# 6Lackiu/EMplanner_Carla

Hardware: AMD Instinct MI355X
Metric: planning cycles/sec (DP+QP, 40x9 S-L lattice, 8 obs) (higher is better)
Workload: dtype f64

## Files before the change

emplanner_carla_amd/csrc/emp_frenet_core.h:

```cpp
#pragma once

#include "emp_core.h"

#if !defined(__HIPCC__)
#include <algorithm>
#endif

namespace emp {

#if !defined(__HIPCC__)
using std::max;
using std::min;
#endif

struct Node {
    double x, y, theta, kappa;
};
EMP_HD Node node_at(const double* line, int i) { return Node{line[4 * i], line[4 * i + 1], line[4 * i + 2], line[4 * i + 3]}; }

EMP_HD int match_scan(const double* line, int n_ref, double x, double y, int first, int step, int limit) {
    int match = 0, worse = 0;
    double best = __builtin_inf();
    for (int i = first; i >= 0 && i < n_ref; i += step) {
        const double dx = line[4 * i] - x, dy = line[4 * i + 1] - y;
        const double d = sqrt(dx * dx + dy * dy);
        if (d < best) {
            best = d;
            match = i;
            worse = 0;
        } else if (++worse >= limit) {
            break;
        }
    }
    return match;
}

EMP_HD double dot2(double a0, double a1, double b0, double b1) { return __builtin_fma(a1, b1, a0 * b0); }

EMP_HD void sincos_pair(double x, double* s, double* c) {
#if defined(__HIP_DEVICE_COMPILE__)
    sincos(x, s, c);
#else
    *s = sin(x);
    *c = cos(x);
#endif
}

EMP_HD Node node_advanced(const Node& m, double ds, double c, double s) {
    return Node{m.x + ds * c, m.y + ds * s, m.theta + m.kappa * ds, m.kappa};
}
EMP_HD void normal_offset(double x, double y, double l, double c, double s, double* ox, double* oy) {
    *ox = x + l * (-s);
    *oy = y + l * c;
}

EMP_HD Node project_on_cs(const Node& m, double c, double s, double x, double y) {
    return node_advanced(m, dot2(x - m.x, y - m.y, c, s), c, s);
}
EMP_HD Node project_on(const Node& m, double x, double y) {
    double c, s;
    sincos_pair(m.theta, &s, &c);
    return project_on_cs(m, c, s, x, y);
}
EMP_HD double projection_s_cs(const Node& m, double c, double s, double s_at_m, double x, double y) {
    return s_at_m + dot2(x - m.x, y - m.y, c, s);
}

EMP_HD double projection_s(const Node& m, double s_at_m, double x, double y) {
    double c, sn;
    sincos_pair(m.theta, &sn, &c);
    return s_at_m + dot2(x - m.x, y - m.y, c, sn);
}

EMP_HD double lateral_offset(const Node& proj, double x, double y) {
    double c, s;
    sincos_pair(proj.theta, &s, &c);
    return dot2(x - proj.x, y - proj.y, -s, c);
}
EMP_HD double lateral_offset_cs(const Node& proj, double c, double s, double x, double y) {
    return dot2(x - proj.x, y - proj.y, -s, c);
}

EMP_HD void s_map_build(const double* line, int n_ref, double ox, double oy, double* s_map) {
    const int m0 = match_scan(line, n_ref, ox, oy, 0, 1, 50);
    double acc = 0.0;
    s_map[0] = 0.0;
    for (int i = 1; i < n_ref; ++i) {
        const double dx = line[4 * i] - line[4 * (i - 1)], dy = line[4 * i + 1] - line[4 * (i - 1) + 1];
        acc = sqrt(dx * dx + dy * dy) + acc;
        s_map[i] = acc;
    }
    const double s0 = projection_s(node_at(line, m0), s_map[m0], ox, oy);
    for (int i = 0; i < n_ref; ++i) s_map[i] = s_map[i] - s0;
}

struct FrenetState {
    double l, l_dot, s_dot, l_ddot, dl_ds, s_ddot, ddl_ds;
};
EMP_HD FrenetState frenet_state_cs(const Node& proj, double c, double s, double px, double py, double vx, double vy, double ax,
                                   double ay) {
    FrenetState o;
    const double k = proj.kappa;
    o.l = dot2(px - proj.x, py - proj.y, -s, c);
    o.l_dot = dot2(vx, vy, -s, c);
    o.s_dot = dot2(vx, vy, c, s) / (1.0 - k * o.l);
    o.l_ddot = dot2(ax, ay, -s, c) - k * (1.0 - k * o.l) * (o.s_dot * o.s_dot);
    o.dl_ds = (fabs(o.s_dot) < 1e-6) ? 0.0 : o.l_dot / o.s_dot;
    o.s_ddot = (dot2(ax, ay, c, s) + 2.0 * (o.s_dot * o.s_dot * k * o.dl_ds) + o.s_dot * o.s_dot * 0.0 * o.l) / (1.0 - k * o.l);
    o.ddl_ds = (fabs(o.s_dot) < 1e-6) ? 0.0 : (o.l_ddot - o.dl_ds * o.s_ddot) / (o.s_dot * o.s_dot);
    return o;
}
EMP_HD FrenetState frenet_state(const Node& proj, double px, double py, double vx, double vy, double ax, double ay) {
    double c, s;
    sincos_pair(proj.theta, &s, &c);
    return frenet_state_cs(proj, c, s, px, py, vx, vy, ax, ay);
}

EMP_HD bool proj_point(const double* line, const double* s_map, int n_ref, double s, int* idx, Node* out) {
    int i = *idx;
    while (true) {
        if (i + 1 >= n_ref) return false;
        if (!(s_map[i + 1] < s)) break;
        ++i;
    }
    const Node m = node_at(line, i);
    const double ds = s - s_map[i];
    double c, sn;
    sincos_pair(m.theta, &sn, &c);
    *out = node_advanced(m, ds, c, sn);
    *idx = i;
    return true;
}

EMP_HD int walk_from_zero(const double* sm, int P, double s, bool* off_end) {
    int lo = 0, hi = P - 1;
    while (lo < hi) {
        const int mid = (lo + hi) >> 1;
        if (sm[mid + 1] < s) lo = mid + 1;
        else hi = mid;
    }
    *off_end = lo + 1 >= P;
    return lo;
}

EMP_HD int argmin_abs(const double* s, int stride, int n, double target) {
    int best = 0;
    double bv = fabs(s[0] - target);
    for (int j = 1; j < n; ++j) {
        const double v = fabs(s[j * stride] - target);
        if (v < bv) {
            bv = v;
            best = j;
        }
    }
    return best;
}

EMP_HD void argmin_abs3(const double* s, int n, double t0, double t1, double t2, int* i0, int* i1, int* i2) {
    const double f = s[0];
    double b0 = fabs(f - t0), b1 = fabs(f - t1), b2 = fabs(f - t2);
    int k0 = 0, k1 = 0, k2 = 0;
    for (int j0 = 1; j0 < n; j0 += 4) {
        double v[4];
#pragma unroll
        for (int u = 0; u < 4; ++u) v[u] = s[min(j0 + u, n - 1)];
#pragma unroll
        for (int u = 0; u < 4; ++u) {
            const int j = j0 + u;
            const double a0 = fabs(v[u] - t0), a1 = fabs(v[u] - t1), a2 = fabs(v[u] - t2);
            if (a0 < b0) { b0 = a0; k0 = j; }
            if (a1 < b1) { b1 = a1; k1 = j; }
            if (a2 < b2) { b2 = a2; k2 = j; }
        }
    }
    *i0 = min(k0, n - 1);
    *i1 = min(k1, n - 1);
    *i2 = min(k2, n - 1);
}

EMP_HD bool lmin_lmax(const double* dp_s, const double* dp_l, int stride, int n, const double* obs_s,
                                 const double* obs_l, int n_obs, double obs_length, double obs_width, double* l_min,
                                 double* l_max) {
    for (int j = 0; j < n; ++j) {
        l_min[j] = -10.0;
        l_max[j] = 10.0;
    }
    for (int k = 0; k < n_obs; ++k) {
        const int lo = argmin_abs(dp_s, stride, n, obs_s[k] - obs_length / 2.0) + 2;
        const int hi = argmin_abs(dp_s, stride, n, obs_s[k] + obs_length / 2.0) + 2;
        const int centre = argmin_abs(dp_s, stride, n, obs_s[k]);
        const bool below = dp_l[centre * stride] < obs_l[k];
        for (int j = lo; j <= hi; ++j) {
            if (j >= n) return false;
            if (below) l_max[j] = fmin(l_max[j], obs_l[k] - obs_width / 2.0);
            else l_min[j] = fmax(l_min[j], obs_l[k] + obs_width / 2.0);
        }
    }
    return true;
}

EMP_HD double centred_diff(const double* v, int stride, int i, int m) {
    const int a = (i - 1 > 0) ? i - 1 : 0, b = (i < m - 2) ? i : m - 2;
    return ((v[(a + 1) * stride] - v[a * stride]) + (v[(b + 1) * stride] - v[b * stride])) / 2.0;
}

EMP_HD void heading_kappa(const double* xy, int stride, int m, double* theta, int tstride, double* kappa, int kstride) {
    for (int i = 0; i < m; ++i) {
        const double dx = centred_diff(xy, stride, i, m), dy = centred_diff(xy + 1, stride, i, m);
        theta[i * tstride] = atan2(dy, dx);
    }
    for (int i = 0; i < m; ++i) {
        const double dx = centred_diff(xy, stride, i, m), dy = centred_diff(xy + 1, stride, i, m);
        kappa[i * kstride] = sin(centred_diff(theta, tstride, i, m)) / sqrt(dx * dx + dy * dy);
    }
}

}
```

emplanner_carla_amd/csrc/emp_qp_rows.h:

```cpp
#pragma once

#include "emp_qp_wave.h"

#ifndef EMP_QP_DEBUG_ROWS
#define EMP_QP_DEBUG_ROWS(...)
#endif

namespace emp {

#pragma clang fp contract(fast)

template <int GP, class Op>
__device__ __forceinline__ double oct_reduce(double v, Op op) {
    static_assert(GP == 8 || GP == 16, "groups of 8 or 16 lanes");
    v = op(v, dpp_move<0xB1>(v));
    v = op(v, dpp_move<0x4E>(v));
    v = op(v, dpp_move<0x141>(v));
    if constexpr (GP == 16) v = op(v, dpp_move<0x140>(v));
    return v;
}
template <int GP>
__device__ __forceinline__ double oct_max(double v) { return oct_reduce<GP>(v, [](double a, double b) { return vmax(a, b); }); }
template <int GP>
__device__ __forceinline__ double oct_min(double v) { return oct_reduce<GP>(v, [](double a, double b) { return vmin(a, b); }); }
// ... 116 lines not shown
        for (int e = 1; e <= KD; ++e) p[e] = lane_up1(y[R - e]);
#pragma unroll
        for (int r = 0; r < R; ++r) {
            double acc = rhs[r];
#pragma unroll
            for (int e = 1; e <= KD; ++e) acc = __builtin_fma(-low[r][e], (r >= e) ? y[r - e] : p[e - r], acc);
            y[r] = acc * rinv[r];
        }
    }
    double x[R];
#pragma unroll
    for (int r = 0; r < R; ++r) x[r] = y[r] * rinv[r];
    for (int k = 0; k < steps; ++k) {
        double q[KD + 1];
#pragma unroll
        for (int e = 1; e <= KD; ++e) q[e] = lane_dn1(x[e - 1]);
#pragma unroll
        for (int r = R - 1; r >= 0; --r) {
            double acc = y[r];
#pragma unroll
            for (int e = 1; e <= KD; ++e) acc = __builtin_fma(-a[r][e], (r + e < R) ? x[r + e] : q[r + e - R + 1], acc);
            x[r] = acc * rinv[r];
        }
    }
#pragma unroll
    for (int r = 0; r < R; ++r) b[r] = x[r];
}

template <int GP, int R>
__device__ __forceinline__ bool band_chol_rows3(double (&a)[R][4], double (&rinv)[R], double (&low)[R][4], int N, int gl,
                                               bool active, int steps) {
    static_assert(R >= 3, "a lane must hold at least KD = 3 rows");
    double A[R][4];
    bool rowv[R], inband[R][4];
#pragma unroll
    for (int r = 0; r < R; ++r) {
        const int j = gl * R + r;
        rowv[r] = active && j < N;
#pragma unroll
        for (int d = 0; d < 4; ++d) {
            A[r][d] = rowv[r] ? a[r][d] : (d == 0 ? 1.0 : 0.0);
            a[r][d] = A[r][d];
            inband[r][d] = rowv[r] && j + d < N;
        }
        rinv[r] = 1.0;
    }
    double diag[R];
    for (int k = 0; k < steps; ++k) {
        const double n1_1 = lane_up1(a[R - 1][1]), n1_2 = lane_up1(a[R - 1][2]), n1_3 = lane_up1(a[R - 1][3]);
        const double n2_2 = lane_up1(a[R - 2][2]), n2_3 = lane_up1(a[R - 2][3]);
        const double n3_3 = lane_up1(a[R - 3][3]);
#pragma unroll
        for (int r = 0; r < R; ++r) {
            double u1_1, u1_2, u1_3, u2_2, u2_3, u3_3;
            if (r >= 1) { u1_1 = a[r - 1][1]; u1_2 = a[r - 1][2]; u1_3 = a[r - 1][3]; }
            else        { u1_1 = n1_1; u1_2 = n1_2; u1_3 = n1_3; }
            if (r >= 2)      { u2_2 = a[r - 2][2]; u2_3 = a[r - 2][3]; }
            else if (r == 1) { u2_2 = n1_2; u2_3 = n1_3; }
            else             { u2_2 = n2_2; u2_3 = n2_3; }
            if (r >= 3)      u3_3 = a[r - 3][3];
            else if (r == 2) u3_3 = n1_3;
            else if (r == 1) u3_3 = n2_3;
            else             u3_3 = n3_3;
            double acc0 = A[r][0], acc1 = A[r][1], acc2 = A[r][2];
            const double acc3 = A[r][3];
            acc0 = __builtin_fma(-u1_1, u1_1, acc0);
            acc1 = __builtin_fma(-u1_1, u1_2, acc1);
            acc2 = __builtin_fma(-u1_1, u1_3, acc2);
            acc0 = __builtin_fma(-u2_2, u2_2, acc0);
            acc1 = __builtin_fma(-u2_2, u2_3, acc1);
            acc0 = __builtin_fma(-u3_3, u3_3, acc0);
            diag[r] = acc0;
            const double rs = fast_rsqrt(acc0 > 0.0 ? acc0 : 1.0);
            a[r][0] = acc0 * rs;
            a[r][1] = inband[r][1] ? acc1 * rs : 0.0;
            a[r][2] = inband[r][2] ? acc2 * rs : 0.0;
            a[r][3] = inband[r][3] ? acc3 * rs : 0.0;
            rinv[r] = rs;
        }
    }
    bool bad = false;
#pragma unroll
    for (int r = 0; r < R; ++r) {
        const double offd = fabs(a[r][1]) + fabs(a[r][2]) + fabs(a[r][3]);
        bad = bad || (rowv[r] && !(diag[r] > 0.0 && diag[r] < 1e300 && offd < 1e300));
    }
    const bool failed = oct_any<GP>(bad);
    if (failed) {
#pragma unroll
        for (int r = 0; r < R; ++r) {
            a[r][0] = 1.0;
            a[r][1] = a[r][2] = a[r][3] = 0.0;
            rinv[r] = 1.0;
        }
    }
    {
        const double n1 = lane_up1(a[R - 1][1]), n1b = lane_up1(a[R - 1][2]), n1c = lane_up1(a[R - 1][3]);
        const double n2b = lane_up1(a[R - 2][2]), n2c = lane_up1(a[R - 2][3]);
        const double n3c = lane_up1(a[R - 3][3]);
        const bool first = gl == 0;
#pragma unroll
        for (int r = 0; r < R; ++r) {
            low[r][0] = 0.0;
            low[r][1] = (r >= 1) ? a[r - 1][1] : (first ? 0.0 : n1);
            low[r][2] = (r >= 2) ? a[r - 2][2] : (r == 1 ? (first ? 0.0 : n1b) : (first ? 0.0 : n2b));
            low[r][3] = (r >= 3) ? a[r - 3][3] : (r == 2 ? (first ? 0.0 : n1c) : (r == 1 ? (first ? 0.0 : n2c) : (first ? 0.0 : n3c)));
        }
    }
    return !failed;
}

template <int R>
__device__ __forceinline__ void band_solve_rows3(const double (&a)[R][4], const double (&rinv)[R], const double (&low)[R][4],
                                                double (&b)[R], int steps) {
    double rhs[R], y[R];
#pragma unroll
    for (int r = 0; r < R; ++r) {
        rhs[r] = (fabs(b[r]) < 1e300) ? b[r] : 0.0;
        y[r] = rhs[r] * rinv[r];
    }
    for (int k = 0; k < steps; ++k) {
        const double p1 = lane_up1(y[R - 1]), p2 = lane_up1(y[R - 2]), p3 = lane_up1(y[R - 3]);
#pragma unroll
        for (int r = 0; r < R; ++r) {
            const double y1 = (r >= 1) ? y[r - 1] : p1;
            const double y2 = (r >= 2) ? y[r - 2] : (r == 1 ? p1 : p2);
            const double y3 = (r >= 3) ? y[r - 3] : (r == 2 ? p1 : (r == 1 ? p2 : p3));
            double acc = __builtin_fma(-low[r][1], y1, rhs[r]);
            acc = __builtin_fma(-low[r][2], y2, acc);
            acc = __builtin_fma(-low[r][3], y3, acc);
            y[r] = acc * rinv[r];
        }
    }
    double x[R];
#pragma unroll
    for (int r = 0; r < R; ++r) x[r] = y[r] * rinv[r];
    for (int k = 0; k < steps; ++k) {
        const double q1 = lane_dn1(x[0]), q2 = lane_dn1(x[1]), q3 = lane_dn1(x[2]);
#pragma unroll
        for (int r = R - 1; r >= 0; --r) {
            const double x1 = (r + 1 < R) ? x[r + 1] : q1;
            const double x2 = (r + 2 < R) ? x[r + 2] : (r + 2 == R ? q1 : q2);
            const double x3 = (r + 3 < R) ? x[r + 3] : (r + 3 == R ? q1 : (r + 3 == R + 1 ? q2 : q3));
            double acc = __builtin_fma(-a[r][1], x1, y[r]);
            acc = __builtin_fma(-a[r][2], x2, acc);
            acc = __builtin_fma(-a[r][3], x3, acc);
            x[r] = acc * rinv[r];
        }
    }
#pragma unroll
    for (int r = 0; r < R; ++r) b[r] = x[r];
}

template <int GP, int R>
__device__ int path_qp_solve_rows(PathRangeQp& Q, int gl, bool live, int iter_cap, double* keep) {
    constexpr int F = 2, W = 3;
    const int N = Q.N, ns = Q.ns, rows = ns * F * 2;
    int state = (live && N > 0) ? 1 : 0;
    int iters = 0;
    bool acceptable = false;
    const int base = gl * R;
    const int steps = oct_wave_max<GP>((state == 1) ? (N + R - 1) / R : 0);
    double g[F][W], gg0[W][F], gg1[W - 1][F], gg2[W - 2][F];
#pragma unroll
    for (int f = 0; f < F; ++f) {
#pragma unroll
        for (int p = 0; p < W; ++p) g[f][p] = wave_uniform(Q.g[f][p]);
    }
#pragma unroll
    for (int f = 0; f < F; ++f) {
#pragma unroll
        for (int p = 0; p < W; ++p) gg0[p][f] = wave_uniform(g[f][p] * g[f][p]);
#pragma unroll
        for (int p = 0; p < W - 1; ++p) gg1[p][f] = wave_uniform(g[f][p] * g[f][p + 1]);
        gg2[0][f] = wave_uniform(g[f][0] * g[f][2]);
    }
    bool tm[R], mm[R], in1[R], in2[R];
#pragma unroll
    for (int r = 0; r < R; ++r) {
        tm[r] = live && base + r < ns;
        mm[r] = live && base + r < N;
        in1[r] = live && base + r + 1 < N;
        in2[r] = live && base + r + 2 < N;
    }
    auto win = [&](const double* vec, double (&out)[R][F]) {
        double vals[R + 2];
#pragma unroll
        for (int i = 0; i < R + 2; ++i) vals[i] = vec[base - 2 + i];
#pragma unroll
        for (int r = 0; r < R; ++r) {
#pragma unroll
            for (int f = 0; f < F; ++f) out[r][f] = (g[f][0] * vals[r] + g[f][1] * vals[r + 1]) + g[f][2] * vals[r + 2];
        }
    };
    auto gather = [&](const double* coef, double (&out)[R]) {
        double cw[R + 2][F];
#pragma unroll
        for (int i = 0; i < R + 2; ++i) {
#pragma unroll
            for (int f = 0; f < F; ++f) cw[i][f] = coef[(base + i) * F + f];
        }
#pragma unroll
        for (int r = 0; r < R; ++r) {
            double acc = 0.0;
#pragma unroll
            for (int p = 0; p < W; ++p) {
#pragma unroll
                for (int f = 0; f < F; ++f) acc += g[f][p] * cw[r + 2 - p][f];
            }
            out[r] = acc;
        }
    };
    auto bounds = [&](double (&c_it)[R][F], double (&lo_it)[R][F], double (&hi_it)[R][F]) {
#pragma unroll
        for (int r = 0; r < R; ++r) {
#pragma unroll
            for (int f = 0; f < F; ++f) {
                c_it[r][f] = Q.c[(base + r) * F + f];
                lo_it[r][f] = Q.lo[(base + r) * F + f];
                hi_it[r][f] = Q.hi[(base + r) * F + f];
            }
        }
    };

    double su[R][F], sl[R][F], zu[R][F], zl[R][F];
    double pdiag = 0.0, qabs = 0.0;
#pragma unroll
    for (int r = 0; r < R; ++r) {
        pdiag = fmax(pdiag, Q.P[(base + r) * 4]);
        qabs = fmax(qabs, fabs(Q.q[base + r]));
    }
    const double pscale = oct_max<GP>(pdiag);
    const double qscale = fmax(oct_max<GP>(qabs), 1.0);
    {
        const double z0 = Q.initial_multiplier(pscale);
        double v[R][F], c_it[R][F], lo_it[R][F], hi_it[R][F];
        bounds(c_it, lo_it, hi_it);
        win(Q.u, v);
        double smin = 1e300;
#pragma unroll
        for (int r = 0; r < R; ++r) {
#pragma unroll
            for (int f = 0; f < F; ++f) {
                zu[r][f] = zl[r][f] = tm[r] ? z0 : 0.0;
                su[r][f] = hi_it[r][f] - (c_it[r][f] + v[r][f]);
                sl[r][f] = (c_it[r][f] + v[r][f]) - lo_it[r][f];
                smin = fmin(smin, fmin(su[r][f], sl[r][f]));
            }
        }
        smin = oct_min<GP>(smin);
        const double shift = (smin < 1.0) ? (1.0 - smin) : 0.0;
#pragma unroll
        for (int r = 0; r < R; ++r) {
#pragma unroll
            for (int f = 0; f < F; ++f) {
                su[r][f] += shift;
                sl[r][f] += shift;
            }
        }
    }

    bool restore = false;
    while (__any(state == 1)) {
        const bool run = state == 1;
        bool acc_now = false;
        double rpu[R][F], rpl[R][F], isu[R][F], isl[R][F], izu[R][F], izl[R][F];
        double rp_max = 0.0, zmax = 0.0, mu = 0.0;
        {
            double v[R][F], c_it[R][F], lo_it[R][F], hi_it[R][F];
            bounds(c_it, lo_it, hi_it);
            win(Q.u, v);
#pragma unroll
            for (int r = 0; r < R; ++r) {
#pragma unroll
                for (int f = 0; f < F; ++f) {
                    rpu[r][f] = (c_it[r][f] + v[r][f]) - hi_it[r][f] + su[r][f];
                    rpl[r][f] = lo_it[r][f] - (c_it[r][f] + v[r][f]) + sl[r][f];
                    isu[r][f] = fast_rcp(su[r][f]);
                    isl[r][f] = fast_rcp(sl[r][f]);
                    izu[r][f] = fast_rcp(zu[r][f]);
                    izl[r][f] = fast_rcp(zl[r][f]);
                    if (tm[r]) {
                        Q.tmp[(base + r) * F + f] = zu[r][f] - zl[r][f];
                        Q.wgt[(base + r) * F + f] = zu[r][f] * isu[r][f] + zl[r][f] * isl[r][f];
                        rp_max = vmax(rp_max, vmax_abs(rpu[r][f], rpl[r][f]));
                        zmax = vmax(zmax, vmax(zu[r][f], zl[r][f]));
                        mu += su[r][f] * zu[r][f] + sl[r][f] * zl[r][f];
                    }
                }
            }
        }
        __syncthreads();
        double rd_m[R], fa[R][4], flow[R][4], frinv[R];
        {
            double ux[R + 6], gz[R];
#pragma unroll
            for (int i = 0; i < R + 6; ++i) ux[i] = Q.u[base - 3 + i];
            gather(Q.tmp, gz);
            double ww[R + 2][F];
#pragma unroll
            for (int i = 0; i < R + 2; ++i) {
#pragma unroll
                for (int f = 0; f < F; ++f) ww[i][f] = Q.wgt[(base + i) * F + f];
            }
            double rd_max = 0.0;
#pragma unroll
            for (int r = 0; r < R; ++r) {
                const int m = base + r;
                double acc = Q.q[m];
#pragma unroll
                for (int d = 0; d < 4; ++d) acc += Q.P[m * 4 + d] * ux[r + 3 + d];
#pragma unroll
                for (int d = 1; d < 4; ++d) acc += Q.P[(m - d) * 4 + d] * ux[r + 3 - d];
                rd_m[r] = mm[r] ? acc + gz[r] : 0.0;
                rd_max = vmax_abs(rd_max, rd_m[r]);
                double e0 = Q.P[m * 4 + 0], e1 = Q.P[m * 4 + 1], e2 = Q.P[m * 4 + 2];
                const double e3 = Q.P[m * 4 + 3];
#pragma unroll
                for (int f = 0; f < F; ++f) {
                    e0 += (ww[r + 2][f] * gg0[0][f] + ww[r + 1][f] * gg0[1][f]) + ww[r][f] * gg0[2][f];
                    e1 += ww[r + 2][f] * gg1[0][f] + ww[r + 1][f] * gg1[1][f];
                    e2 += ww[r + 2][f] * gg2[0][f];
                }
                fa[r][0] = e0;
                fa[r][1] = in1[r] ? e1 : 0.0;
                fa[r][2] = in2[r] ? e2 : 0.0;
                fa[r][3] = e3;
            }
            rd_max = oct_max<GP>(rd_max);
            rp_max = oct_max<GP>(rp_max);
            zmax = oct_max<GP>(zmax);
            mu = oct_sum<GP>(mu) / (double)rows;
            if (run) {
                const double dscale = fmax(qscale, zmax);
                if (rd_max <= Q.eps_d_rel * dscale && rp_max <= Q.eps_p && mu <= Q.eps_mu) state = 0;
                else if (!(mu == mu) || mu > 1e30 || (iters >= kQpStallIter && rp_max > kQpStallResidual)) state = 2;
                else if (rp_max > kQpStallResidual && zmax > kQpInfeasibleZ * pscale) state = 2;
                else if (iters >= kQpMaxIter || iters >= iter_cap) state = acceptable ? 0 : 2;
                acc_now = rd_max <= 100.0 * Q.eps_d_rel * dscale && rp_max <= 10.0 * Q.eps_p && mu <= 1000.0 * Q.eps_mu;
                if (acc_now) acceptable = true;
                if (state == 1 && acc_now && rp_max <= Q.eps_p && mu <= Q.eps_mu) state = 0;
                if (state == 0 && acceptable && !acc_now) restore = true;
                EMP_QP_DEBUG_ROWS("R it %d rd %.3e rp %.3e mu %.3e zmax %.3e -> state %d acc %d\n", iters, rd_max, rp_max, mu, zmax, state, (int)acceptable);
            }
        }
        if (run && acc_now) {
#pragma unroll
            for (int r = 0; r < R; ++r)
                if (mm[r]) keep[base + r] = Q.u[base + r];
        }
        if (!__any(state == 1)) break;
        const bool go = state == 1;
#ifdef EMP_QP_PROBE_SKIP_CHOL
        bool okf = true;
#pragma unroll
        for (int r = 0; r < R; ++r) {
            frinv[r] = (go && mm[r]) ? 1.0 / (fa[r][0] + 1.0) : 1.0;
#pragma unroll
            for (int d = 0; d < 4; ++d) flow[r][d] = 0.0;
        }
#else
        const bool okf = band_chol_rows3<GP, R>(fa, frinv, flow, N, gl, go, steps);
#endif
        EMP_QP_DEBUG_ROWS("R    chol ok %d\n", (int)okf);
        if (go && !okf) {
            state = acceptable ? 0 : 2;
            if (acceptable && !acc_now) restore = true;
        }
        const bool go2 = state == 1;
#pragma unroll
        for (int r = 0; r < R; ++r) {
            if (tm[r]) {
#pragma unroll
                for (int f = 0; f < F; ++f)
                    Q.tmp[(base + r) * F + f] = -(((zu[r][f] * isu[r][f]) * rpu[r][f] - zu[r][f]) - ((zl[r][f] * isl[r][f]) * rpl[r][f] - zl[r][f]));
            }
        }
        __syncthreads();
        double dua[R];
        gather(Q.tmp, dua);
#pragma unroll
        for (int r = 0; r < R; ++r) dua[r] = (go2 && mm[r]) ? (-rd_m[r] + dua[r]) : 0.0;
#ifndef EMP_QP_PROBE_SKIP_SOLVE
        band_solve_rows3<R>(fa, frinv, flow, dua, steps);
#endif
#pragma unroll
        for (int r = 0; r < R; ++r)
            if (mm[r]) Q.dua[base + r] = dua[r];
        __syncthreads();
        double rcu[R][F], rcl[R][F];
        {
            double gda[R][F], dsua[R][F], dsla[R][F], dzua[R][F], dzla[R][F];
            win(Q.dua, gda);
            double ratio = 0.0;
#pragma unroll
            for (int r = 0; r < R; ++r) {
                const bool ok = tm[r];
#pragma unroll
                for (int f = 0; f < F; ++f) {
                    dsua[r][f] = -rpu[r][f] - gda[r][f];
                    dsla[r][f] = -rpl[r][f] + gda[r][f];
                    dzua[r][f] = -zu[r][f] - (zu[r][f] * isu[r][f]) * dsua[r][f];
                    dzla[r][f] = -zl[r][f] - (zl[r][f] * isl[r][f]) * dsla[r][f];
                    if (ok)
                        ratio = vmax(ratio, vmax(vmax(-dsua[r][f] * isu[r][f], -dsla[r][f] * isl[r][f]),
                                                 vmax(-dzua[r][f] * izu[r][f], -dzla[r][f] * izl[r][f])));
                }
            }
            ratio = oct_max<GP>(ratio);
            const double a_aff = (ratio > 1.0) ? fast_rcp(ratio) : 1.0;
            double mu_aff = 0.0;
#pragma unroll
            for (int r = 0; r < R; ++r) {
#pragma unroll
                for (int f = 0; f < F; ++f)
                    mu_aff += (su[r][f] + a_aff * dsua[r][f]) * (zu[r][f] + a_aff * dzua[r][f]) +
                              (sl[r][f] + a_aff * dsla[r][f]) * (zl[r][f] + a_aff * dzla[r][f]);
            }
            mu_aff = oct_sum<GP>(mu_aff) / (double)rows;
            double sigma = (mu > 0.0) ? mu_aff * fast_rcp(mu) : 0.0;
            sigma = sigma * sigma * sigma;
#pragma unroll
            for (int r = 0; r < R; ++r) {
                const bool ok = tm[r];
#pragma unroll
                for (int f = 0; f < F; ++f) {
                    rcu[r][f] = su[r][f] * zu[r][f] + dsua[r][f] * dzua[r][f] - sigma * mu;
                    rcl[r][f] = sl[r][f] * zl[r][f] + dsla[r][f] * dzla[r][f] - sigma * mu;
                }
                if (ok) {
#pragma unroll
                    for (int f = 0; f < F; ++f)
                        Q.tmp[(base + r) * F + f] = -((zu[r][f] * rpu[r][f] - rcu[r][f]) * isu[r][f] - (zl[r][f] * rpl[r][f] - rcl[r][f]) * isl[r][f]);
                }
            }
        }
        __syncthreads();
        double du[R];
        gather(Q.tmp, du);
#pragma unroll
        for (int r = 0; r < R; ++r) du[r] = (go2 && mm[r]) ? (-rd_m[r] + du[r]) : 0.0;
#ifndef EMP_QP_PROBE_SKIP_SOLVE
        band_solve_rows3<R>(fa, frinv, flow, du, steps);
#endif
#pragma unroll
        for (int r = 0; r < R; ++r)
            if (mm[r]) Q.rhs[base + r] = du[r];
        __syncthreads();
        {
            double gd[R][F], dsu[R][F], dsl[R][F], dzu[R][F], dzl[R][F];
            win(Q.rhs, gd);
            double ratio = 0.0;
#pragma unroll
            for (int r = 0; r < R; ++r) {
                const bool ok = tm[r];
#pragma unroll
                for (int f = 0; f < F; ++f) {
                    dsu[r][f] = -rpu[r][f] - gd[r][f];
                    dsl[r][f] = -rpl[r][f] + gd[r][f];
                    dzu[r][f] = -(rcu[r][f] + zu[r][f] * dsu[r][f]) * isu[r][f];
                    dzl[r][f] = -(rcl[r][f] + zl[r][f] * dsl[r][f]) * isl[r][f];
                    if (ok)
                        ratio = vmax(ratio, vmax(vmax(-dsu[r][f] * isu[r][f], -dsl[r][f] * isl[r][f]),
                                                 vmax(-dzu[r][f] * izu[r][f], -dzl[r][f] * izl[r][f])));
                }
            }
            ratio = oct_max<GP>(ratio);
            const double tau = qp_step_fraction(mu);
            const double alpha = (ratio > tau) ? tau * fast_rcp(ratio) : 1.0;
            EMP_QP_DEBUG_ROWS("R    alpha %.6e\n", alpha);
            if (go2) {
#pragma unroll
                for (int r = 0; r < R; ++r) {
                    if (tm[r]) {
#pragma unroll
                        for (int f = 0; f < F; ++f) {
                            su[r][f] += alpha * dsu[r][f];
                            sl[r][f] += alpha * dsl[r][f];
                            zu[r][f] += alpha * dzu[r][f];
                            zl[r][f] += alpha * dzl[r][f];
                        }
                    }
                    if (mm[r]) Q.u[base + r] = Q.u[base + r] + alpha * du[r];
                }
                ++iters;
            }
        }
        __syncthreads();
    }
    if (restore) {
#pragma unroll
        for (int r = 0; r < R; ++r)
            if (mm[r]) Q.u[base + r] = keep[base + r];
    }
    __syncthreads();
    Q.iters = iters;
    return state;
}

template <int GP, int R>
__host__ __device__ constexpr int path_qp_words_rows() { return PathQpRowsLayout<GP, R>::words; }

template <int GP, int R>
__device__ __forceinline__ void path_qp_pad_rows(double* lds, int N, int ns, int gl) {
    PathQpRowsLayout<GP, R>::pad_ranges(N, ns, [&](int first, int last, double v) {
        for (int i = first + gl; i < last; i += GP) lds[i] = v;
    });
}

template <int GP, int R>
__device__ inline int path_qp_group_rows(double* lds, const double* l_min, const double* l_max, int n, double l0, double dl0,
                                         double ddl0, const PathQpParams& prm, double* out_l, int* iters_out, bool live,
                                         int debug_stage = 0) {
    using L = PathQpRowsLayout<GP, R>;
    const int gl = (threadIdx.x & 63) & (GP - 1);
    *iters_out = 0;
    PathRangeQp Q;
    double* cc = lds + L::cc;
    const int nn = live ? n : 4;
    Q.N = nn - 4 > 0 ? nn - 4 : 0;
    Q.ns = nn - 2 > 0 ? nn - 2 : 0;
    Q.P = lds + L::P;
    Q.q = lds + L::q;
    Q.u = lds + L::u;
    Q.dua = lds + L::dua;
    Q.rhs = lds + L::rhs;
    Q.c = lds + L::c;
    Q.lo = lds + L::lo;
    Q.hi = lds + L::hi;
    Q.tmp = lds + L::tmp;
    Q.wgt = lds + L::wgt;
    int rc = path_qp_setup_group<GP>(Q, cc, l_min, l_max, n, l0, dl0, ddl0, prm, gl, live);
    if (!live) rc = 2;
    if (EMP_DEV_HOOKS && debug_stage == 2) rc = 2;
    __syncthreads();
    bool ok = rc == 0;
    const int base = gl * R;
    {
        double fa[R][4], flow[R][4], frinv[R], b0[R];
        const bool act = ok && Q.N > 0;
        const int steps = oct_wave_max<GP>(act ? (Q.N + R - 1) / R : 0);
#pragma unroll
        for (int r = 0; r < R; ++r) {
            const bool has = act && base + r < Q.N;
#pragma unroll
            for (int d = 0; d < 4; ++d) {
                const double raw = Q.P[(base + r) * 4 + d];
                fa[r][d] = has ? raw : 0.0;
            }
            const double qr = Q.q[base + r];
            b0[r] = has ? -qr : 0.0;
        }
        const bool okc = band_chol_rows3<GP, R>(fa, frinv, flow, Q.N, gl, act, steps);
        band_solve_rows3<R>(fa, frinv, flow, b0, steps);
#pragma unroll
        for (int r = 0; r < R; ++r)
            if (act && base + r < Q.N) Q.u[base + r] = b0[r];
        if (ok && !okc) rc = 2;
    }
    if (EMP_DEV_HOOKS && debug_stage == 3) rc = 2;
    ok = rc == 0;
    path_qp_pad_rows<GP, R>(lds, ok ? Q.N : 0, ok ? Q.ns : 0, gl);
    __syncthreads();
    const int cap_it = debug_stage >= 10 ? debug_stage - 10 : 1000;
    const int rs = path_qp_solve_rows<GP, R>(Q, gl, ok && Q.N > 0, cap_it, cc + 3);
    if (ok && Q.N > 0) {
        *iters_out = Q.iters;
        if (rs && (debug_stage < 10 || !EMP_DEV_HOOKS)) rc = rs;
    }
    ok = rc == 0;
    if (ok && Q.N == 0) {
        bool bad = false;
        for (int it = gl; it < Q.ns * 2; it += GP)
            if (Q.c[it] > Q.hi[it] + 1e-9 || Q.c[it] < Q.lo[it] - 1e-9) bad = true;
        if (oct_any<GP>(bad)) rc = 1;
    }
    ok = rc == 0;
    for (int m = gl; m < (ok ? Q.N : 0); m += GP) cc[m + 3] = Q.u[m];
    __syncthreads();
    for (int i = gl; i < (ok ? n : 0); i += GP) out_l[i] = (cc[i] + 4.0 * cc[i + 1] + cc[i + 2]) / 6.0;
    __syncthreads();
    return rc;
}

#pragma clang fp contract(off)

}
```

emplanner_carla_amd/csrc/emp_tail_kernels.h:

```cpp
#pragma once

#include <hip/hip_runtime.h>

#include "emp_core.h"
#include "emp_frenet_core.h"
#include "emp_qp_core.h"
#include "emp_qp_wave.h"
#include "emp_qp_rows.h"
#include "emp_smooth_rows.h"
#include "emp_tail_launch.h"

namespace emp {

constexpr int kStDpInfeasible = 1, kStSOutOfRange = 2, kStBoundIndex = 4, kStQpFailed = 8, kStSmoothFailed = 16,
              kStTruncated = 32;

struct QpDev {
    PathQpParams qp;
    double obs_length, obs_width;
    int decimate, midpoint, use_qp;
    int debug_stage;
};

template <int CTRL, int ROW_MASK>
// ... 327 lines not shown
                                                         SmoothQpParams sy, const double* __restrict__ xy,
                                                         const int* __restrict__ n_pts, double* __restrict__ out,
                                                         int* __restrict__ iters, int* __restrict__ status) {
    extern __shared__ __attribute__((aligned(16))) double lds[];
    const int b = blockIdx.x;
    const int m = min(max(n_pts[b], 0), max_pts);
    int it = 0, rc = 2;
    double *px = nullptr, *py = nullptr;
    if (m <= cap) rc = smooth_pair_wave<WIDE>(smooth_lds(lds, m).qmem, xy + (size_t)b * max_pts * 2, 2, m, sx, sy, &px, &py, &it);
    if (rc == 0) heading_kappa_lanes<64>(px, py, m, smooth_lds(lds, m).theta, out + (size_t)b * max_pts * 4, 4);
    if ((threadIdx.x & 63) == 0) {
        if (iters) iters[b] = it;
        status[b] = rc ? kStSmoothFailed : 0;
    }
}

__global__ __launch_bounds__(64) void reference_line_wave_kernel(int B, int max_global, SmoothQpParams sx, SmoothQpParams sy,
                                                                 const double* __restrict__ global_path,
                                                                 const int* __restrict__ n_global,
                                                                 const double* __restrict__ pred_xy,
                                                                 const int* __restrict__ is_first_run,
                                                                 const int* __restrict__ pre_match_index,
                                                                 double* __restrict__ ref_line, int* __restrict__ n_ref,
                                                                 int* __restrict__ match_index, int* __restrict__ iters,
                                                                 int* __restrict__ status, int n_ref_on_fail = 0) {
    extern __shared__ __attribute__((aligned(16))) double lds[];
    const int b = blockIdx.x, lane = threadIdx.x & 63;
    const double* line = global_path + (size_t)b * max_global * 4;
    const int P = min(n_global[b], max_global);
    const RefLineLds<double*> L = ref_line_lds(lds);
    double* gxy = L.gxy;
    double* qmem = L.smooth.qmem;
    double* out = ref_line + (size_t)b * kRefLinePoints * 4;
    int m = 0, first = 0, fail = 0;
    if (lane == 0) {
        const double x = pred_xy[2 * b], y = pred_xy[2 * b + 1];
        const int st = pre_match_index[b];
        if (P < 1 || ((!is_first_run || !is_first_run[b]) && (st < 0 || st >= P))) {
            fail = kStSOutOfRange;
        } else {
            m = find_match_one(line, P, x, y, !(is_first_run && is_first_run[b]), st);
        }
        int back = 10, fwd = 40;
        if (m < back) {
            back = m;
            fwd = 50 - back;
        }
        if (P - m - 1 < fwd) {
            fwd = P - m - 1;
            back = 50 - fwd;
        }
        first = m - back;
        if (!fail && (first < 0 || m + fwd + 1 > P)) fail = kStSOutOfRange;
    }
    m = __shfl(m, 0, 64);
    first = __shfl(first, 0, 64);
    fail = __shfl(fail, 0, 64);
    int it = 0;
    if (!fail) {
        if (lane < kRefLinePoints) {
            gxy[2 * lane] = line[4 * (first + lane)];
            gxy[2 * lane + 1] = line[4 * (first + lane) + 1];
        }
        __syncthreads();
        double *px = nullptr, *py = nullptr;
        const int rc = smooth_pair_wave<true>(qmem, gxy, 2, kRefLinePoints, sx, sy, &px, &py, &it);
        if (rc) fail = kStSmoothFailed;
        else heading_kappa_lanes<64>(px, py, kRefLinePoints, L.smooth.theta, out, 4);
    }
    if (fail)
        for (int i = lane; i < kRefLinePoints * 4; i += 64) out[i] = 0.0;
    if (lane == 0) {
        n_ref[b] = fail ? n_ref_on_fail : kRefLinePoints;
        match_index[b] = m;
        if (iters) iters[b] = it;
        status[b] = fail;
    }
}

__device__ inline int frenet_path_to_xy(const double* line, const double* s_map, int P, double begin_s, double begin_l,
                                        const double* path_s, const double* path_l, int n, double* target_xy,
                                        int cap, bool* s_error, bool* trunc) {
    *s_error = false;
    *trunc = false;
    int idx = 0, m = 0;
    Node pr;
    if (!proj_point(line, s_map, P, begin_s, &idx, &pr)) {
        *s_error = true;
        return 0;
    }
    double pc, psn;
    sincos_pair(pr.theta, &psn, &pc);
    normal_offset(pr.x, pr.y, begin_l, pc, psn, &target_xy[0], &target_xy[1]);
    m = 1;
    for (int i = 0; i < n; ++i) {
        const double s = path_s[i];
        if (s > s_map[P - 1]) break;
        if (!proj_point(line, s_map, P, s, &idx, &pr)) {
            *s_error = true;
            return m;
        }
        if (m >= cap) {
            *trunc = true;
            break;
        }
        sincos_pair(pr.theta, &psn, &pc);
        normal_offset(pr.x, pr.y, path_l[i], pc, psn, &target_xy[2 * m], &target_xy[2 * m + 1]);
        ++m;
    }
    return m;
}

__global__ void path_to_xy_kernel(int B, int max_ref, int max_pts, const double* __restrict__ ref_line,
                                  const double* __restrict__ s_map, const int* __restrict__ n_ref,
                                  const double* __restrict__ begin_sl, const double* __restrict__ path_s,
                                  const double* __restrict__ path_l, const int* __restrict__ n_pts,
                                  double* __restrict__ target_xy, int* __restrict__ n_out, int* __restrict__ status) {
    const int b = blockIdx.x * blockDim.x + threadIdx.x;
    if (b >= B) return;
    const int P = min(max(n_ref[b], 0), max_ref);
    const int n = min(max(n_pts[b], 0), max_pts);
    bool s_err, trunc;
    const int m = frenet_path_to_xy(ref_line + (size_t)b * max_ref * 4, s_map + (size_t)b * max_ref, P,
                                    begin_sl[2 * b], begin_sl[2 * b + 1], path_s + (size_t)b * max_pts,
                                    path_l + (size_t)b * max_pts, n, target_xy + (size_t)b * (max_pts + 1) * 2,
                                    max_pts + 1, &s_err, &trunc);
    n_out[b] = m;
    status[b] = (s_err ? kStSOutOfRange : 0) | (trunc ? kStTruncated : 0);
}

template <int G, int R = 0>
__host__ __device__ constexpr int cycle_qp_group_words(int cap, int max_obs) {
    if (R > 0) return PathQpRowsLayout<(R > 0 ? G : 8), (R > 0 ? R : 3)>::stride(max_obs);
    return cycle_qp_lds(0, G == 32, cap, max_obs).end;
}
template <int G, int R = 0>
__device__ __forceinline__ void cycle_qp_body(int B, int max_pts, int max_obs, int cap, const QpDev& Q,
                                                           const double* __restrict__ dp_s,
                                                           const double* __restrict__ dp_l,
                                                           const int* __restrict__ dp_len,
                                                           const double* __restrict__ obs_s,
                                                           const double* __restrict__ obs_l,
                                                           const int* __restrict__ n_obs,
                                                           const double* __restrict__ start,
                                                           double* __restrict__ path_s, double* __restrict__ path_l,
                                                           int* __restrict__ path_len, int* __restrict__ status) {
    extern __shared__ __attribute__((aligned(16))) double lds_all[];
    __builtin_amdgcn_s_setprio(EMP_PRIO_BACK);
    constexpr int GPW = 64 / G;
    const int lane = threadIdx.x & 63, grp = lane / G, gl = lane & (G - 1);
    const int b = blockIdx.x * GPW + grp;
    const bool present = b < B;
    static_assert(R == 0 || G == 8 || G == 16, "the rows solver runs on groups of 8 or 16 lanes");
    const int per_group = cycle_qp_group_words<G, R>(cap, max_obs);
    double* lds = lds_all + (size_t)grp * per_group;
    const size_t o = (size_t)(present ? b : 0) * max_pts;
    double* sd = lds;
    double *ld, *lmin, *lmax, *ql, *otab, *qmem;
    if constexpr (R > 0) {
        using L = PathQpRowsLayout<G, R>;
        qmem = lds;
        ql = qmem + L::result;
        sd = qmem + L::path;
        ld = sd + cap;
        lmin = ld + cap;
        lmax = lmin + cap;
        otab = qmem + (max_obs <= L::C ? L::obstacles : L::words);
    } else {
        const CycleQpLds<double*> L = cycle_qp_lds(lds, G == 32, cap, max_obs);
        ld = L.ld;
        lmin = L.lmin;
        lmax = L.lmax;
        ql = L.ql;
        otab = L.otab;
        qmem = L.qmem;
    }
#ifdef EMP_QP_PROBE_EMPTY
    if (Q.debug_stage == 4) return;
#endif
    const int ne = present ? dp_len[b] : 0;
    const int dec = Q.decimate > 0 ? Q.decimate : 1;
    const int n = (ne + dec - 1) / dec;
    const int st = present ? status[b] : 0;
    int fail = 0;
    if (present && (n > cap || n + (Q.midpoint ? 1 : 0) > max_pts || n < 1)) fail = kStTruncated;
    bool live = present && !fail;
    for (int i = gl; i < (live ? n : 0); i += G) {
        sd[i] = dp_s[o + (size_t)i * dec];
        ld[i] = dp_l[o + (size_t)i * dec];
    }
    __syncthreads();
#ifdef EMP_QP_PROBE_EMPTY
    if (Q.debug_stage == 5) return;
#endif
    if (Q.use_qp) {
        const int nob = live ? min(max(n_obs[b], 0), max_obs) : 0;
        bool bad = false;
        for (int k = gl; k < nob; k += G) {
            const double os = obs_s[(size_t)b * max_obs + k], ol = obs_l[(size_t)b * max_obs + k];
            int lo, hi, centre;
            argmin_abs3(sd, n, os - Q.obs_length / 2.0, os + Q.obs_length / 2.0, os, &lo, &hi, &centre);
            lo += 2;
            hi += 2;
            const bool below = ld[centre] < ol;
            otab[4 * k + 0] = (double)lo;
            otab[4 * k + 1] = (double)hi;
            otab[4 * k + 2] = below ? 1.0 : 0.0;
            otab[4 * k + 3] = below ? ol - Q.obs_width / 2.0 : ol + Q.obs_width / 2.0;
            if (lo <= hi && hi >= n) bad = true;
        }
        if (group_any<G>(bad) && live) {
            fail = kStBoundIndex;
            live = false;
        }
        __syncthreads();
        {
            constexpr int T = R > 0 ? R + 1 : (G == 64 ? 4 : 2);
            const int nn = live ? n : 0;
            double a[T], c[T];
#pragma unroll
            for (int t = 0; t < T; ++t) {
                a[t] = -10.0;
                c[t] = 10.0;
            }
            for (int k = 0; k < nob; ++k) {
                const double klo = otab[4 * k], khi = otab[4 * k + 1], kbelow = otab[4 * k + 2], kb = otab[4 * k + 3];
#pragma unroll
                for (int t = 0; t < T; ++t) {
                    const double j = (double)(gl + G * t);
                    if (j >= klo && j <= khi) {
                        if (kbelow != 0.0) c[t] = fmin(c[t], kb);
                        else a[t] = fmax(a[t], kb);
                    }
                }
            }
#pragma unroll
            for (int t = 0; t < T; ++t) {
                const int j = gl + G * t;
                if (j < nn) {
                    lmin[j] = a[t];
                    lmax[j] = c[t];
                }
            }
            for (int j = gl + G * T; j < nn; j += G) {
                double aj = -10.0, cj = 10.0;
                for (int k = 0; k < nob; ++k) {
                    if ((double)j >= otab[4 * k] && (double)j <= otab[4 * k + 1]) {
                        if (otab[4 * k + 2] != 0.0) cj = fmin(cj, otab[4 * k + 3]);
                        else aj = fmax(aj, otab[4 * k + 3]);
                    }
                }
                lmin[j] = aj;
                lmax[j] = cj;
            }
        }
        __syncthreads();
        if (Q.debug_stage == 1) live = false;
        int it = 0;
        const int sb = present ? b : 0;
        int rc;
        if constexpr (R > 0)
            rc = path_qp_group_rows<G, R>(qmem, lmin, lmax, n, start[4 * sb + 1], start[4 * sb + 2], start[4 * sb + 3], Q.qp, ql, &it,
                                       live, Q.debug_stage);
        else
            rc = path_qp_group<G>(qmem, lmin, lmax, n, start[4 * sb + 1], start[4 * sb + 2], start[4 * sb + 3], Q.qp,
                                  ql, nullptr, nullptr, &it, live, Q.debug_stage);
        if (live && rc) {
            fail = kStQpFailed;
            live = false;
        }
    } else {
        for (int i = gl; i < (live ? n : 0); i += G) ql[i] = ld[i];
        __syncthreads();
    }
    if (present) {
        double* ps = path_s + o;
        double* pl = path_l + o;
        int plen = 0;
        auto sd_at = [&](int i) {
            if constexpr (R > 0) return dp_s[o + (size_t)i * dec];
            else return sd[i];
        };
        if (live) {
            if (Q.midpoint) {
                for (int i = gl; i <= n; i += G) {
                    if (i == 0) {
                        ps[0] = sd_at(0);
                        pl[0] = ql[0];
                    } else if (i == n) {
                        ps[n] = sd_at(n - 1);
                        pl[n] = ql[n - 1];
                    } else {
                        ps[i] = (sd_at(i) + sd_at(i - 1)) / 2.0;
                        pl[i] = (ql[i] + ql[i - 1]) / 2.0;
                    }
                }
                plen = n + 1;
            } else {
                for (int i = gl; i < n; i += G) {
                    ps[i] = sd_at(i);
                    pl[i] = ql[i];
                }
                plen = n;
            }
        }
        for (int i = plen + gl; i < max_pts; i += G) {
            ps[i] = 0.0;
            pl[i] = 0.0;
        }
        if (gl == 0) {
            path_len[b] = plen;
            status[b] = st | fail;
        }
    }
}

#define EMP_CYCLE_QP_PARAMS                                                                                         \
    int B, int max_pts, int max_obs, int cap, QpDev Q, const double *__restrict__ dp_s, const double *__restrict__ dp_l, \
        const int *__restrict__ dp_len, const double *__restrict__ obs_s, const double *__restrict__ obs_l,           \
        const int *__restrict__ n_obs, const double *__restrict__ start, double *__restrict__ path_s,                  \
        double *__restrict__ path_l, int *__restrict__ path_len, int *__restrict__ status
#define EMP_CYCLE_QP_ARGS B, max_pts, max_obs, cap, Q, dp_s, dp_l, dp_len, obs_s, obs_l, n_obs, start, path_s, path_l, path_len, status
template <int G>
__global__ __launch_bounds__(64) void cycle_qp_wave_kernel(EMP_CYCLE_QP_PARAMS) {
    cycle_qp_body<G>(EMP_CYCLE_QP_ARGS);
}
template <int GP, int R>
__global__ __launch_bounds__(64) void cycle_qp_rows_kernel(EMP_CYCLE_QP_PARAMS) {
    cycle_qp_body<GP, R>(EMP_CYCLE_QP_ARGS);
}
#undef EMP_CYCLE_QP_PARAMS
#undef EMP_CYCLE_QP_ARGS


#define EMP_CARTESIAN_PARAMS                                                                                                       \
    int B, int max_ref, int max_pts, int cap, SmoothQpParams sx, SmoothQpParams sy, const double *__restrict__ ref_line,            \
        const double *__restrict__ s_map, const int *__restrict__ n_ref, const double *__restrict__ begin_sl,                       \
        const double *__restrict__ path_s, const double *__restrict__ path_l, const int *__restrict__ path_len,                     \
        double *__restrict__ traj, int *__restrict__ traj_len, int *__restrict__ status
#define EMP_CARTESIAN_ARGS B, max_ref, max_pts, cap, sx, sy, ref_line, s_map, n_ref, begin_sl, path_s, path_l, path_len, traj, traj_len, status
template <int SL, int R, bool WIDE>
__device__ __forceinline__ void cycle_cartesian_body(EMP_CARTESIAN_PARAMS, int force_fallback) {
    extern __shared__ __attribute__((aligned(16))) double lds[];
    __builtin_amdgcn_s_setprio(EMP_PRIO_CART);
    constexpr int GP = SL / 2, SPW = 64 / SL;
    static_assert(R > 0 ? (SL == 16 || SL == 32) : SL == 64, "rows smoother: 16 or 32 lanes per scene; else the whole wavefront");
    const int lane = threadIdx.x & 63, sc = lane / SL, sl = lane & (SL - 1);
    const int b = blockIdx.x * SPW + sc;
    const bool present = b < B;
    const size_t bb = present ? (size_t)b : 0;
    const int per_scene = cartesian_scene_lds(0, max_ref, cap).end;
    double *sm, *txy, *th, *px, *py, *qmem;
    if constexpr (R > 0) {
        const CartesianSceneLds<double*> L = cartesian_scene_lds(lds + (size_t)sc * per_scene, max_ref, cap);
        sm = L.sm;
        txy = L.txy;
        th = L.th;
        px = L.px;
        py = L.py;
        qmem = lds + (size_t)SPW * per_scene;
    } else {
        const CartesianLds<double*> L = cartesian_lds(lds, max_ref, cap);
        sm = L.sm;
        txy = L.txy;
        th = L.th;
        qmem = L.qmem;
        px = py = nullptr;
    }
    const int st = present ? status[bb] : 0;
    int add = 0;
    bool alive = present && !(st & (kStQpFailed | kStBoundIndex | kStTruncated));
    const double* line = ref_line + bb * max_ref * 4;
    const int P = present ? min(max(n_ref[bb], 0), max_ref) : 0;
    const int n = alive ? path_len[bb] : 0;
    for (int i = sl; i < P; i += SL) sm[i] = s_map[bb * max_ref + i];
    __syncthreads();
    bool off = false;
    const double bs = present ? begin_sl[2 * bb] : 0.0, bl = alive ? begin_sl[2 * bb + 1] : 0.0;
    const int idx0 = walk_from_zero(sm, P, bs, &off);
    if (present && (off || P < 2)) {
        add = kStSOutOfRange;
        alive = false;
    }
    const double s_last = alive ? sm[P - 1] : 0.0;
    int carry = idx0, count = alive ? n : 0;
    bool stop = !alive;
    int qmax = 0;
#pragma unroll
    for (int g = 0; g < SPW; ++g) qmax = max(qmax, __builtin_amdgcn_readlane(alive ? n + 1 : 0, SL * g));
    constexpr unsigned long long kSceneMask = ~0ull >> (64 - SL);
    for (int base = 0; base < qmax; base += SL) {
        const int q = base + sl, i = q - 1;
        const bool is0 = alive && q == 0;
        const bool in = !stop && i >= 0 && i < n;
        const double s = in ? path_s[bb * max_pts + i] : 0.0;
        const unsigned long long bad = (__ballot(in && s > s_last) >> (SL * sc)) & kSceneMask;
        const int first_bad = SL == 64 ? __builtin_ffsll((long long)bad) : __builtin_ffs((int)bad);
        if (!stop && first_bad) count = min(count, base + first_bad - 2);
        bool o2 = false;
        int k = in ? walk_from_zero(sm, P, fmin(s, s_last), &o2) : 0;
        for (int d = 1; d < SL; d <<= 1) {
            const int v = __shfl_up(k, d, SL);
            if (sl >= d) k = max(k, v);
        }
        k = max(k, carry);
        carry = __shfl(k, SL - 1, SL);
        if (is0 || (in && i < count && i + 1 < cap)) {
            const Node mm = node_at(line, k);
            const double ds = (is0 ? bs : s) - sm[k], l = is0 ? bl : path_l[bb * max_pts + i];
            double mc, msn, pc, psn;
            sincos_pair(mm.theta, &msn, &mc);
            const Node pr = node_advanced(mm, ds, mc, msn);
            sincos_pair(pr.theta, &psn, &pc);
            normal_offset(pr.x, pr.y, l, pc, psn, &txy[2 * q], &txy[2 * q + 1]);
        }
        if (first_bad) stop = true;
    }
    int m = count + 1;
    __syncthreads();
    if (alive && (m > cap || m > max_pts + 1 || (R > 0 && m > GP * R))) {
        add = kStTruncated;
        alive = false;
    }
    if (alive && m < 2) {
        add = kStSmoothFailed;
        alive = false;
// ... 301 lines not shown
```

Before: 19.24 million.

## Replace block barriers with wavefront-scoped LDS ordering in rows QP solver

Swaps __syncthreads in the row-based QP solver and the tail kernel for a wavefront fence plus wave barrier, relying on each solver group living inside one wavefront. It also hoists the per-scene global loads (obs count, first obstacle, start state) ahead of the first barrier and adds asm register pins and local copies of u. The aim is to drop block-wide barrier cost and hide global load latency. If a group ever spans wavefronts, or another group's data is touched, ordering could break.

```diff
diff --git a/emplanner_carla_amd/csrc/emp_frenet_core.h b/emplanner_carla_amd/csrc/emp_frenet_core.h
--- a/emplanner_carla_amd/csrc/emp_frenet_core.h
+++ b/emplanner_carla_amd/csrc/emp_frenet_core.h
@@ -173,9 +173,9 @@
             if (a2 < b2) { b2 = a2; k2 = j; }
         }
     }
-    *i0 = min(k0, n - 1);
-    *i1 = min(k1, n - 1);
-    *i2 = min(k2, n - 1);
+    *i0 = max(min(k0, n - 1), 0);
+    *i1 = max(min(k1, n - 1), 0);
+    *i2 = max(min(k2, n - 1), 0);
 }
 
 EMP_HD bool lmin_lmax(const double* dp_s, const double* dp_l, int stride, int n, const double* obs_s,
diff --git a/emplanner_carla_amd/csrc/emp_qp_rows.h b/emplanner_carla_amd/csrc/emp_qp_rows.h
--- a/emplanner_carla_amd/csrc/emp_qp_rows.h
+++ b/emplanner_carla_amd/csrc/emp_qp_rows.h
@@ -292,6 +292,12 @@
     for (int r = 0; r < R; ++r) b[r] = x[r];
 }
 
+__device__ __forceinline__ void rows_lds_order() {
+    __builtin_amdgcn_fence(__ATOMIC_RELEASE, "wavefront");
+    __builtin_amdgcn_wave_barrier();
+    __builtin_amdgcn_fence(__ATOMIC_ACQUIRE, "wavefront");
+}
+
 template <int GP, int R>
 __device__ int path_qp_solve_rows(PathRangeQp& Q, int gl, bool live, int iter_cap, double* keep) {
     constexpr int F = 2, W = 3;
@@ -430,7 +436,7 @@
                 }
             }
         }
-        __syncthreads();
+        rows_lds_order();
         double rd_m[R], fa[R][4], flow[R][4], frinv[R];
         {
             double ux[R + 6], gz[R];
@@ -452,7 +458,9 @@
                 for (int d = 0; d < 4; ++d) acc += Q.P[m * 4 + d] * ux[r + 3 + d];
 #pragma unroll
                 for (int d = 1; d < 4; ++d) acc += Q.P[(m - d) * 4 + d] * ux[r + 3 - d];
-                rd_m[r] = mm[r] ? acc + gz[r] : 0.0;
+                double rd = acc + gz[r];
+                asm volatile("" : "+v"(rd));
+                rd_m[r] = mm[r] ? rd : 0.0;
                 rd_max = vmax_abs(rd_max, rd_m[r]);
                 double e0 = Q.P[m * 4 + 0], e1 = Q.P[m * 4 + 1], e2 = Q.P[m * 4 + 2];
                 const double e3 = Q.P[m * 4 + 3];
@@ -485,9 +493,14 @@
             }
         }
         if (run && acc_now) {
+            double uk[R];
+#pragma unroll
+            for (int r = 0; r < R; ++r) uk[r] = Q.u[base + r];
+#pragma unroll
+            for (int r = 0; r < R; ++r) asm volatile("" : "+v"(uk[r]));
 #pragma unroll
             for (int r = 0; r < R; ++r)
-                if (mm[r]) keep[base + r] = Q.u[base + r];
+                if (mm[r]) keep[base + r] = uk[r];
         }
         if (!__any(state == 1)) break;
         const bool go = state == 1;
@@ -516,7 +529,7 @@
                     Q.tmp[(base + r) * F + f] = -(((zu[r][f] * isu[r][f]) * rpu[r][f] - zu[r][f]) - ((zl[r][f] * isl[r][f]) * rpl[r][f] - zl[r][f]));
             }
         }
-        __syncthreads();
+        rows_lds_order();
         double dua[R];
         gather(Q.tmp, dua);
 #pragma unroll
@@ -527,7 +540,7 @@
 #pragma unroll
         for (int r = 0; r < R; ++r)
             if (mm[r]) Q.dua[base + r] = dua[r];
-        __syncthreads();
+        rows_lds_order();
         double rcu[R][F], rcl[R][F];
         {
             double gda[R][F], dsua[R][F], dsla[R][F], dzua[R][F], dzla[R][F];
@@ -575,7 +588,7 @@
                 }
             }
         }
-        __syncthreads();
+        rows_lds_order();
         double du[R];
         gather(Q.tmp, du);
 #pragma unroll
@@ -586,10 +599,15 @@
 #pragma unroll
         for (int r = 0; r < R; ++r)
             if (mm[r]) Q.rhs[base + r] = du[r];
-        __syncthreads();
+        rows_lds_order();
         {
             double gd[R][F], dsu[R][F], dsl[R][F], dzu[R][F], dzl[R][F];
             win(Q.rhs, gd);
+            double uo[R];
+#pragma unroll
+            for (int r = 0; r < R; ++r) uo[r] = Q.u[base + r];
+#pragma unroll
+            for (int r = 0; r < R; ++r) asm volatile("" : "+v"(uo[r]));
             double ratio = 0.0;
 #pragma unroll
             for (int r = 0; r < R; ++r) {
@@ -621,19 +639,19 @@
                             zl[r][f] += alpha * dzl[r][f];
                         }
                     }
-                    if (mm[r]) Q.u[base + r] = Q.u[base + r] + alpha * du[r];
+                    if (mm[r]) Q.u[base + r] = uo[r] + alpha * du[r];
                 }
                 ++iters;
             }
         }
-        __syncthreads();
+        rows_lds_order();
     }
     if (restore) {
 #pragma unroll
         for (int r = 0; r < R; ++r)
             if (mm[r]) Q.u[base + r] = keep[base + r];
     }
-    __syncthreads();
+    rows_lds_order();
     Q.iters = iters;
     return state;
 }
@@ -673,7 +691,7 @@
     int rc = path_qp_setup_group<GP>(Q, cc, l_min, l_max, n, l0, dl0, ddl0, prm, gl, live);
     if (!live) rc = 2;
     if (EMP_DEV_HOOKS && debug_stage == 2) rc = 2;
-    __syncthreads();
+    rows_lds_order();
     bool ok = rc == 0;
     const int base = gl * R;
     {
@@ -701,7 +719,7 @@
     if (EMP_DEV_HOOKS && debug_stage == 3) rc = 2;
     ok = rc == 0;
     path_qp_pad_rows<GP, R>(lds, ok ? Q.N : 0, ok ? Q.ns : 0, gl);
-    __syncthreads();
+    rows_lds_order();
     const int cap_it = debug_stage >= 10 ? debug_stage - 10 : 1000;
     const int rs = path_qp_solve_rows<GP, R>(Q, gl, ok && Q.N > 0, cap_it, cc + 3);
     if (ok && Q.N > 0) {
@@ -717,9 +735,9 @@
     }
     ok = rc == 0;
     for (int m = gl; m < (ok ? Q.N : 0); m += GP) cc[m + 3] = Q.u[m];
-    __syncthreads();
+    rows_lds_order();
     for (int i = gl; i < (ok ? n : 0); i += GP) out_l[i] = (cc[i] + 4.0 * cc[i + 1] + cc[i + 2]) / 6.0;
-    __syncthreads();
+    rows_lds_order();
     return rc;
 }
 
diff --git a/emplanner_carla_amd/csrc/emp_tail_kernels.h b/emplanner_carla_amd/csrc/emp_tail_kernels.h
--- a/emplanner_carla_amd/csrc/emp_tail_kernels.h
+++ b/emplanner_carla_amd/csrc/emp_tail_kernels.h
@@ -503,6 +503,10 @@
     const int b = blockIdx.x * GPW + grp;
     const bool present = b < B;
     static_assert(R == 0 || G == 8 || G == 16, "the rows solver runs on groups of 8 or 16 lanes");
+    auto lds_sync = [] {
+        if constexpr (R > 0) rows_lds_order();
+        else __syncthreads();
+    };
     const int per_group = cycle_qp_group_words<G, R>(cap, max_obs);
     double* lds = lds_all + (size_t)grp * per_group;
     const size_t o = (size_t)(present ? b : 0) * max_pts;
@@ -529,10 +533,25 @@
 #ifdef EMP_QP_PROBE_EMPTY
     if (Q.debug_stage == 4) return;
 #endif
-    const int ne = present ? dp_len[b] : 0;
+    const int sb = present ? b : 0;
+    const int ne_scene = dp_len[sb], st_scene = status[sb];
+    int nob_scene = 0;
+    double os_first = 0.0, ol_first = 0.0, start_l = 0.0, start_dl = 0.0, start_ddl = 0.0;
+    if (Q.use_qp) {
+        nob_scene = n_obs[sb];
+        if (max_obs > 0) {
+            const size_t slot = (size_t)sb * max_obs + min(gl, max_obs - 1);
+            os_first = obs_s[slot];
+            ol_first = obs_l[slot];
+        }
+        start_l = start[4 * sb + 1];
+        start_dl = start[4 * sb + 2];
+        start_ddl = start[4 * sb + 3];
+    }
+    const int ne = present ? ne_scene : 0;
+    const int st = present ? st_scene : 0;
     const int dec = Q.decimate > 0 ? Q.decimate : 1;
     const int n = (ne + dec - 1) / dec;
-    const int st = present ? status[b] : 0;
     int fail = 0;
     if (present && (n > cap || n + (Q.midpoint ? 1 : 0) > max_pts || n < 1)) fail = kStTruncated;
     bool live = present && !fail;
@@ -540,15 +559,16 @@
         sd[i] = dp_s[o + (size_t)i * dec];
         ld[i] = dp_l[o + (size_t)i * dec];
     }
-    __syncthreads();
+    lds_sync();
 #ifdef EMP_QP_PROBE_EMPTY
     if (Q.debug_stage == 5) return;
 #endif
     if (Q.use_qp) {
-        const int nob = live ? min(max(n_obs[b], 0), max_obs) : 0;
+        const int nob = live ? min(max(nob_scene, 0), max_obs) : 0;
         bool bad = false;
         for (int k = gl; k < nob; k += G) {
-            const double os = obs_s[(size_t)b * max_obs + k], ol = obs_l[(size_t)b * max_obs + k];
+            const bool first = k == gl;
+            const double os = first ? os_first : obs_s[(size_t)b * max_obs + k], ol = first ? ol_first : obs_l[(size_t)b * max_obs + k];
             int lo, hi, centre;
             argmin_abs3(sd, n, os - Q.obs_length / 2.0, os + Q.obs_length / 2.0, os, &lo, &hi, &centre);
             lo += 2;
@@ -564,7 +584,7 @@
             fail = kStBoundIndex;
             live = false;
         }
-        __syncthreads();
+        lds_sync();
         {
             constexpr int T = R > 0 ? R + 1 : (G == 64 ? 4 : 2);
             const int nn = live ? n : 0;
@@ -574,6 +594,7 @@
                 a[t] = -10.0;
                 c[t] = 10.0;
             }
+#pragma unroll 4
             for (int k = 0; k < nob; ++k) {
                 const double klo = otab[4 * k], khi = otab[4 * k + 1], kbelow = otab[4 * k + 2], kb = otab[4 * k + 3];
 #pragma unroll
@@ -605,24 +626,22 @@
                 lmax[j] = cj;
             }
         }
-        __syncthreads();
+        lds_sync();
         if (Q.debug_stage == 1) live = false;
         int it = 0;
-        const int sb = present ? b : 0;
         int rc;
         if constexpr (R > 0)
-            rc = path_qp_group_rows<G, R>(qmem, lmin, lmax, n, start[4 * sb + 1], start[4 * sb + 2], start[4 * sb + 3], Q.qp, ql, &it,
-                                       live, Q.debug_stage);
+            rc = path_qp_group_rows<G, R>(qmem, lmin, lmax, n, start_l, start_dl, start_ddl, Q.qp, ql, &it, live, Q.debug_stage);
         else
-            rc = path_qp_group<G>(qmem, lmin, lmax, n, start[4 * sb + 1], start[4 * sb + 2], start[4 * sb + 3], Q.qp,
-                                  ql, nullptr, nullptr, &it, live, Q.debug_stage);
+            rc = path_qp_group<G>(qmem, lmin, lmax, n, start_l, start_dl, start_ddl, Q.qp, ql, nullptr, nullptr, &it, live,
+                                  Q.debug_stage);
         if (live && rc) {
             fail = kStQpFailed;
             live = false;
         }
     } else {
         for (int i = gl; i < (live ? n : 0); i += G) ql[i] = ld[i];
-        __syncthreads();
+        lds_sync();
     }
     if (present) {
         double* ps = path_s + o;
```

Result: no change. 19.23 million (-0.1%).
